# MasonFeurer/VoxelRayTracing

Hardware: AMD Instinct MI355X
Metric: Mrays/s at 1920x1080, 1 primary + 1 shadow ray (higher is better)
Workload: dtype f32

## Files before the change

bindings/rust/vrt-sys/src/lib.rs:

```rust
#![allow(non_camel_case_types)]
use std::os::raw::{c_char, c_int, c_void};

#[repr(C)]
pub struct vrt_ctx {
    _private: [u8; 0],
}

pub const VRT_OK: c_int = 0;
pub const VRT_ERR_INVALID_ARG: c_int = -1;
pub const VRT_ERR_OUT_OF_RANGE: c_int = -2;
pub const VRT_ERR_DEVICE: c_int = -3;
pub const VRT_ERR_OOM: c_int = -4;
pub const VRT_ERR_STATE: c_int = -5;

#[repr(C)]
#[derive(Clone, Copy, Default)]
pub struct vrt_material {
    pub color: [f32; 3],
    pub is_empty: u32,
    pub is_liquid: u32,
    pub scatter: f32,
    pub _padding: [u32; 2],
}

// ... 396 lines not shown
    pub fn vrt_read_tone_histogram(ctx: *mut vrt_ctx, bins: *mut u32) -> c_int;
    pub fn vrt_set_sun_light(ctx: *mut vrt_ctx, opts: *const vrt_sun_light) -> c_int;
    pub fn vrt_set_camera_sampling(ctx: *mut vrt_ctx, opts: *const vrt_camera_sampling) -> c_int;
    pub fn vrt_set_lamp_light(ctx: *mut vrt_ctx, opts: *const vrt_lamp_light) -> c_int;
    pub fn vrt_get_lamp_info(ctx: *mut vrt_ctx, out: *mut vrt_lamp_info) -> c_int;
    pub fn vrt_read_lamps(ctx: *mut vrt_ctx, out: *mut vrt_lamp, cap: u32, n: *mut u32) -> c_int;
    pub fn vrt_synchronize(ctx: *mut vrt_ctx) -> c_int;
    pub fn vrt_read_output(ctx: *mut vrt_ctx, rgb: *mut f32, ids: *mut u32, rgba8: *mut u8) -> c_int;
    pub fn vrt_present(ctx: *mut vrt_ctx, crosshair: *const vrt_crosshair, screen_w: u32, screen_h: u32, rgba8: *mut u8) -> c_int;
    pub fn vrt_selftest_exact_math(device: i32, n: u32, seed: u32, mismatches: *mut u64) -> c_int;
    pub fn vrt_selftest_math_values(device: i32, op: u32, n: u32, input: *const u32, out: *mut u32) -> c_int;
    pub fn vrt_present_device(ctx: *mut vrt_ctx, crosshair: *const vrt_crosshair, screen_w: u32, screen_h: u32, rgba8_device: *mut *mut c_void, bytes: *mut u64) -> c_int;
    pub fn vrt_set_presentation(ctx: *mut vrt_ctx, crosshair: *const vrt_crosshair, screen_w: u32, screen_h: u32, flags: u32) -> c_int;
    pub fn vrt_get_stats(ctx: *mut vrt_ctx, out: *mut vrt_stats) -> c_int;
    pub fn vrt_get_issue_profile(ctx: *mut vrt_ctx, out: *mut vrt_issue_profile) -> c_int;
    pub fn vrt_get_accel_info(ctx: *mut vrt_ctx, out: *mut vrt_accel_info) -> c_int;
    pub fn vrt_read_accel(ctx: *mut vrt_ctx, grid: *mut u32, bricks: *mut u16) -> c_int;
    pub fn vrt_read_march_cells(ctx: *mut vrt_ctx, cells: *mut u32, direct: *mut u32) -> c_int;
    pub fn vrt_read_tile_cost(ctx: *mut vrt_ctx, cost: *mut u32) -> c_int;
    pub fn vrt_read_tile_order(ctx: *mut vrt_ctx, order: *mut u32, dilated: *mut u32) -> c_int;
    pub fn vrt_selftest_tile_order(device: i32, cost: *const u32, tiles_x: u32, tiles_y: u32, radius: i32, order: *mut u32) -> c_int;
    pub fn vrt_get_sun_marks(ctx: *mut vrt_ctx, passes: *mut u32, min_leaf: *mut u32, lit_trips: *mut u32, lit: *mut u8) -> c_int;
    pub fn vrt_read_lit_voxels(ctx: *mut vrt_ctx, passes: *mut u32, layers: *mut u32, lit_trips: *mut u32, lit: *mut u8) -> c_int;
    pub fn vrt_get_dark_marks(ctx: *mut vrt_ctx, passes: *mut u32, count: *mut u32, used: *mut u32, dark: *mut u8) -> c_int;
    pub fn vrt_read_steps(ctx: *mut vrt_ctx, steps: *mut u32) -> c_int;
    pub fn vrt_set_stream(ctx: *mut vrt_ctx, hip_stream: *mut c_void) -> c_int;
    pub fn vrt_bind_output(ctx: *mut vrt_ctx, texels: *mut c_void) -> c_int;
    pub fn vrt_device_output(ctx: *mut vrt_ctx, texels: *mut *mut c_void, bytes: *mut u64) -> c_int;
    pub fn vrt_shard_info(ctx: *mut vrt_ctx, tiles_local: *mut u32, tiles_padded: *mut u32, tiles_total: *mut u32) -> c_int;
    pub fn vrt_assemble(ctx: *mut vrt_ctx, gathered: *const c_void, rank_stride_bytes: u64, dst: *mut c_void) -> c_int;
    pub fn vrt_assemble_compact(ctx: *mut vrt_ctx, gathered: *const c_void, rank_stride_bytes: u64, dst: *mut c_void) -> c_int;
    pub fn vrt_cast_rays(ctx: *mut vrt_ctx, queries: *const vrt_ray_query, n: u32, out: *mut vrt_ray_hit) -> c_int;
    pub fn vrt_cast_rays_device(ctx: *mut vrt_ctx, queries_device: *const c_void, n: u32, out_device: *mut c_void) -> c_int;
    pub fn vrt_clip_moves(ctx: *mut vrt_ctx, queries: *const vrt_box_query, n: u32, out: *mut vrt_box_move) -> c_int;
    pub fn vrt_clip_moves_device(ctx: *mut vrt_ctx, queries_device: *const c_void, n: u32, out_device: *mut c_void) -> c_int;
    pub fn vrt_get_voxels(ctx: *mut vrt_ctx, pos: *const i32, n: u32, out: *mut vrt_voxel_at) -> c_int;
    pub fn vrt_get_voxels_device(ctx: *mut vrt_ctx, pos_device: *const c_void, n: u32, out_device: *mut c_void) -> c_int;
    pub fn vrt_column_tops(ctx: *mut vrt_ctx, queries: *const vrt_column_query, n: u32, out: *mut vrt_column_top) -> c_int;
    pub fn vrt_column_tops_device(ctx: *mut vrt_ctx, queries_device: *const c_void, n: u32, out_device: *mut c_void) -> c_int;
    pub fn vrt_read_top_map(ctx: *mut vrt_ctx, flags: u32, map: *mut vrt_top_entry) -> c_int;
    pub fn vrt_top_map_device(ctx: *mut vrt_ctx, flags: u32, map_device: *mut c_void) -> c_int;
    pub fn vrt_generate_chunks(ctx: *mut vrt_ctx, seed: u32, chunk_pos: *const i32, n: u32, nodes: *mut u16, cap_nodes: u64,
                               offsets: *mut u64) -> c_int;
    pub fn vrt_build_chunks(ctx: *mut vrt_ctx, dense: *const u16, n: u32, nodes: *mut u16, cap_nodes: u64, offsets: *mut u64) -> c_int;
    pub fn vrt_edit_chunks(ctx: *mut vrt_ctx, chunk_pos: *const i32, n: u32, nodes_in: *const u16, offsets_in: *const u64,
                           shapes: *const vrt_shape, m: u32, nodes_out: *mut u16, cap_nodes: u64, offsets_out: *mut u64,
// ... 33 lines not shown
```

include/vrt.h:

```cpp
#ifndef VRT_H
#define VRT_H

#include <stdint.h>

#ifdef __cplusplus
extern "C" {
#endif

typedef struct vrt_ctx vrt_ctx;

typedef enum {
    VRT_OK = 0,
    VRT_ERR_INVALID_ARG = -1,
    VRT_ERR_OUT_OF_RANGE = -2,
    VRT_ERR_DEVICE = -3,
    VRT_ERR_OOM = -4,
    VRT_ERR_STATE = -5
} vrt_status;

typedef struct {
    float color[3];
    uint32_t is_empty;
    uint32_t is_liquid;
    float scatter;
// ... 272 lines not shown
int vrt_selftest_math_values(int32_t device, uint32_t op, uint32_t n, const uint32_t *in, uint32_t *out);

typedef struct {
    uint32_t available;
    uint32_t world_size_chunks;
    uint64_t cells;
    uint64_t bricks;
    uint64_t bytes;
    uint32_t builds;
    float last_build_ms;
    uint32_t chunk_builds;
    uint32_t ordered_frames;
} vrt_accel_info;
int vrt_get_accel_info(vrt_ctx *ctx, vrt_accel_info *out);

int vrt_read_accel(vrt_ctx *ctx, uint32_t *grid, uint16_t *bricks);

int vrt_read_march_cells(vrt_ctx *ctx, uint32_t *cells, uint32_t *direct);

int vrt_get_sun_marks(vrt_ctx *ctx, uint32_t *passes, uint32_t *min_leaf, uint32_t *lit_trips, uint8_t *lit);

int vrt_read_lit_voxels(vrt_ctx *ctx, uint32_t *passes, uint32_t *layers, uint32_t *lit_trips, uint8_t *lit);

int vrt_get_dark_marks(vrt_ctx *ctx, uint32_t *passes, uint32_t *count, uint32_t *used, uint8_t *dark);

int vrt_read_tile_cost(vrt_ctx *ctx, uint32_t *cost);

int vrt_read_tile_order(vrt_ctx *ctx, uint32_t *order, uint32_t *dilated);

int vrt_selftest_tile_order(int32_t device, const uint32_t *cost, uint32_t tiles_x, uint32_t tiles_y, int32_t radius, uint32_t *order);

int vrt_read_steps(vrt_ctx *ctx, uint32_t *steps);


typedef struct {
    float start[3];
    float max_dist;
    float dir[3];
    uint32_t _reserved;
} vrt_ray_query;

#define VRT_RAY_MISS 0u
#define VRT_RAY_HIT 1u
#define VRT_RAY_REJECTED 2u
typedef struct {
    int32_t pos[3];
// ... 116 lines not shown
```

voxelraytracing_amd/_ffi.py:

```python
from __future__ import annotations

import ctypes as C
import os

import numpy as np

_HERE = os.path.dirname(os.path.abspath(__file__))


class Material(C.Structure):
    _fields_ = [("color", C.c_float * 3), ("is_empty", C.c_uint32), ("is_liquid", C.c_uint32),
                ("scatter", C.c_float), ("_padding", C.c_uint32 * 2)]


class CamData(C.Structure):
    _fields_ = [("pos", C.c_float * 3), ("_padding0", C.c_uint32), ("inv_view_mat", C.c_float * 16),
                ("inv_proj_mat", C.c_float * 16), ("proj_size", C.c_float * 2), ("_padding1", C.c_uint32 * 2)]


class WorldData(C.Structure):
    _fields_ = [("min", C.c_int32 * 3), ("size", C.c_uint32), ("size_in_chunks", C.c_uint32),
                ("_padding", C.c_uint32 * 3)]


# ... 199 lines not shown
    "vrt_read_guide": (C.c_int, [_P, _P]),
    "vrt_set_tone_map": (C.c_int, [_P, C.POINTER(ToneMap)]),
    "vrt_get_tone_info": (C.c_int, [_P, C.POINTER(ToneInfo)]),
    "vrt_read_tone_histogram": (C.c_int, [_P, _P]),
    "vrt_set_sun_light": (C.c_int, [_P, C.POINTER(SunLight)]),
    "vrt_set_camera_sampling": (C.c_int, [_P, C.POINTER(CameraSampling)]),
    "vrt_set_lamp_light": (C.c_int, [_P, C.POINTER(LampLight)]),
    "vrt_get_lamp_info": (C.c_int, [_P, C.POINTER(LampInfo)]),
    "vrt_read_lamps": (C.c_int, [_P, _P, C.c_uint32, C.POINTER(C.c_uint32)]),
    "vrt_synchronize": (C.c_int, [_P]),
    "vrt_read_output": (C.c_int, [_P, _P, _P, _P]),
    "vrt_present": (C.c_int, [_P, C.POINTER(Crosshair), C.c_uint32, C.c_uint32, _P]),
    "vrt_selftest_exact_math": (C.c_int, [C.c_int32, C.c_uint32, C.c_uint32, C.POINTER(C.c_uint64)]),
    "vrt_selftest_math_values": (C.c_int, [C.c_int32, C.c_uint32, C.c_uint32, _P, _P]),
    "vrt_present_device": (C.c_int, [_P, C.POINTER(Crosshair), C.c_uint32, C.c_uint32, C.POINTER(_P), C.POINTER(C.c_uint64)]),
    "vrt_set_presentation": (C.c_int, [_P, C.POINTER(Crosshair), C.c_uint32, C.c_uint32, C.c_uint32]),
    "vrt_get_stats": (C.c_int, [_P, C.POINTER(Stats)]),
    "vrt_get_issue_profile": (C.c_int, [_P, C.POINTER(IssueProfile)]),
    "vrt_get_accel_info": (C.c_int, [_P, C.POINTER(AccelInfo)]),
    "vrt_read_accel": (C.c_int, [_P, _P, _P]),
    "vrt_read_march_cells": (C.c_int, [_P, _P, _P]),
    "vrt_get_sun_marks": (C.c_int, [_P, _P, _P, _P, _P]),
    "vrt_read_lit_voxels": (C.c_int, [_P, _P, _P, _P, _P]),
    "vrt_get_dark_marks": (C.c_int, [_P, _P, _P, _P, _P]),
    "vrt_read_tile_cost": (C.c_int, [_P, _P]),
    "vrt_read_tile_order": (C.c_int, [_P, _P, C.POINTER(C.c_uint32)]),
    "vrt_selftest_tile_order": (C.c_int, [C.c_int32, _P, C.c_uint32, C.c_uint32, C.c_int32, _P]),
    "vrt_read_steps": (C.c_int, [_P, _P]),
    "vrt_set_stream": (C.c_int, [_P, _P]),
    "vrt_bind_output": (C.c_int, [_P, _P]),
    "vrt_device_output": (C.c_int, [_P, C.POINTER(_P), C.POINTER(C.c_uint64)]),
    "vrt_shard_info": (C.c_int, [_P, C.POINTER(C.c_uint32), C.POINTER(C.c_uint32), C.POINTER(C.c_uint32)]),
    "vrt_assemble": (C.c_int, [_P, _P, C.c_uint64, _P]),
    "vrt_assemble_compact": (C.c_int, [_P, _P, C.c_uint64, _P]),
    "vrt_cast_rays": (C.c_int, [_P, _P, C.c_uint32, _P]),
    "vrt_cast_rays_device": (C.c_int, [_P, _P, C.c_uint32, _P]),
    "vrt_clip_moves": (C.c_int, [_P, _P, C.c_uint32, _P]),
    "vrt_clip_moves_device": (C.c_int, [_P, _P, C.c_uint32, _P]),
    "vrt_get_voxels": (C.c_int, [_P, _P, C.c_uint32, _P]),
    "vrt_get_voxels_device": (C.c_int, [_P, _P, C.c_uint32, _P]),
    "vrt_column_tops": (C.c_int, [_P, _P, C.c_uint32, _P]),
    "vrt_column_tops_device": (C.c_int, [_P, _P, C.c_uint32, _P]),
    "vrt_read_top_map": (C.c_int, [_P, C.c_uint32, _P]),
    "vrt_top_map_device": (C.c_int, [_P, C.c_uint32, _P]),
    "vrt_generate_chunks": (C.c_int, [_P, C.c_uint32, _P, C.c_uint32, _P, C.c_uint64, _P]),
    "vrt_build_chunks": (C.c_int, [_P, _P, C.c_uint32, _P, C.c_uint64, _P]),
# ... 200 lines not shown
```

voxelraytracing_amd/csrc/vrt_ctx.h:

```cpp
#pragma once
#include <hip/hip_runtime.h>

#include <algorithm>
#include <array>
#include <atomic>
#include <condition_variable>
#include <functional>
#include <memory>
#include <mutex>
#include <thread>
#include <cmath>
#include <cstdarg>
#include <cstdio>
#include <cstdlib>
#include <cstring>
#include <new>
#include <string>
#include <vector>

#include "vrt_devbuf.h"
#include "vrt_frame_plan.h"
#include "vrt_handle.h"
#include "vrt_device.h"

// ... 194 lines not shown
        uint64_t gen = 0;
        struct SunMarks {
            struct Key {
                uint64_t gen = 0;
                float sun[3] = {0.f, 0.f, 0.f};
                uint32_t min_lo = 0;
                uint32_t liquid[8] = {0, 0, 0, 0, 0, 0, 0, 0};
                bool same(const Key &o) const {
                    return gen == o.gen && memcmp(sun, o.sun, sizeof sun) == 0 && min_lo == o.min_lo && memcmp(liquid, o.liquid, sizeof liquid) == 0;
                }
            } made, want;
            uint32_t want_frames = 0;
            bool valid = false;
            Buf<uint16_t> d_pool;
            Buf<uint32_t> d_clash;
            bool voxels_valid = false;
            uint64_t pool_gen = ~0ull;
            Pinned h_clash;
            bool clash_pending = false;
            uint64_t clash_gen = ~0ull;
            uint32_t voxel_layers = 0;
            Buf<uint8_t> d_floors;
            bool dark_valid = false;
            Event ev;
            bool pending = false;
            hipStream_t stream = nullptr;
            Event ev_guard;
            bool holds(uint64_t gen) const { return valid && made.gen == gen; }
            bool pool_fits(size_t entries) const { return d_pool && d_pool.cap() == entries; }
            bool pool_is_of(uint64_t gen, size_t entries) const { return pool_gen == gen && holds(gen) && pool_fits(entries); }
            void take_from(const SunMarks &A, uint64_t a_gen, uint64_t gen) {
                valid = A.holds(a_gen);
                made = A.made; made.gen = gen;
                pending = voxels_valid = false;
                dark_valid = valid && A.dark_valid;
            }
        } lit;
        Event ev_updated;
        bool update_pending = false;
    };
    Tables tabs[kMaxInFlight];
    uint64_t tables_gen = 0;
    bool tables_split = false;
    uint32_t quiet_frames = 0;
    bool shared_readers_in_flight = false;
    Buf<uint32_t> d_brick_total;
// ... 3 lines not shown
    uint32_t n_bricks = 0;
    uint32_t accel_S = 0;
    bool accel_dirty = true;
    bool accel_ok = false;
    uint32_t accel_max_s = 0;
    uint32_t timing_every = 8, frame_no = 0;
    bool path_pool = true;
    bool path_cells = true;
    uint32_t path_samples = 8;
    uint32_t path_pool_batches = 0;
    uint32_t path_refill = 0;
    uint32_t accel_builds = 0;
    bool sun_marks = true;
    uint32_t lit_slab = 0;
    uint32_t lit_passes = 0;
    bool lit_voxels = true;
    int lit_voxel_layers = -1;
    uint32_t lit_voxel_passes = 0;
    uint32_t lit_last_voxel_layers = 0, lit_last_voxel_trips = 0;
    uint32_t lit_last_min_leaf = 0, lit_last_trips = 0;
    bool dark_marks = true;
    int dark_depth = -1;
    uint32_t dark_passes = 0;
    bool dark_last_used = false;
    bool tile_lpt = true;
    uint32_t view_gen = 0;
    uint32_t frame_view_gen = ~0u;
    uint32_t order_view_gen = ~0u;
    uint32_t tile_lpt_moving = 1;
    uint32_t order_uses = 0;
    uint32_t mov_backoff = 0, mov_skip = 0;
    bool mov_any_size = false;
    uint32_t mov_radius = 5;
    uint32_t one_w = 0, one_h = 0;
    bool one_to_one = false;
    bool pres_on = false;
    vrt_crosshair pres_ch{};
    uint32_t pres_w = 0, pres_h = 0, pres_flags = 0;
    uint32_t pres_for_w = 0, pres_for_h = 0, pres_box[4] = {0, 0, 0, 0};
    bool pres_fusable = false;
    uint32_t ordered_frames = 0;
    bool order_dilated = false;
    uint32_t cam_gen = 0, order_cam_gen = 0;
    vrt_cam_data order_cam{};
    bool tile_order_stale = false;
    uint32_t frame_mode = ~0u;
// ... 290 lines not shown
```

voxelraytracing_amd/csrc/vrt_device.h:

```cpp
#pragma once

#include <hip/hip_runtime.h>
#include <stddef.h>
#include <stdint.h>

#include "../../include/vrt.h"

namespace vrt {

constexpr float kShadowBias = 0.002f;
constexpr float kShadowFactor = 0.35f;
constexpr uint32_t kMaxSteps = 500u;
constexpr uint32_t kIdNormYNeg = 1u << 23;

constexpr uint32_t kCamNotFinite = 1u, kCamOnPlane = 2u, kCamOutside = 4u;

constexpr uint32_t kAirLeaf = 0xFF800000u;
__host__ __device__ inline bool is_split_entry(uint32_t e) { return (int32_t)e < 0 && e < kAirLeaf; }
constexpr uint32_t kAirUnlit = 1u << 22;
constexpr uint32_t kLitBelow = kAirLeaf | kAirUnlit;
constexpr uint32_t kAirDark = 1u << 21;
constexpr uint32_t kLitVoxel = 0x7FFFu;
__host__ __device__ inline uint32_t grid_entry(uint32_t x) { return x - 1u < 31u ? (kAirLeaf | kAirUnlit | x) : x; }

using Texel = uint4;

constexpr uint32_t kMaterials = 256u;
__host__ __device__ inline const float *emission_table(const vrt_material *mats) { return reinterpret_cast<const float *>(mats + kMaterials); }
__host__ __device__ inline const vrt_polish *polish_table(const vrt_material *mats) {
    return reinterpret_cast<const vrt_polish *>(emission_table(mats) + kMaterials);
}
static_assert(sizeof(vrt_polish) == 32 && (kMaterials * (sizeof(vrt_material) + sizeof(float))) % 16 == 0, "the polish table's entries are 16-byte aligned");
__host__ __device__ inline const vrt_translucency *translucency_table(const vrt_material *mats) {
    return reinterpret_cast<const vrt_translucency *>(polish_table(mats) + kMaterials);
}
__host__ __device__ inline const uint32_t *coat_word(const vrt_material *mats) {
    return reinterpret_cast<const uint32_t *>(translucency_table(mats) + kMaterials);
}
static_assert(sizeof(vrt_translucency) == 16, "a translucency entry is one 16-byte load");

struct FrameParams {
    const uint16_t *nodes;
    const uint32_t *roots;
    const vrt_material *mats;
    const uint32_t *grid;
// ... 174 lines not shown
```

voxelraytracing_amd/csrc/vrt_frames.hip:

```cpp
#include "vrt_ctx.h"

thread_local std::string g_create_err;

int fail(vrt_ctx *ctx, int code, const char *fmt, ...) {
    char buf[512];
    va_list ap;
    va_start(ap, fmt);
    vsnprintf(buf, sizeof buf, fmt, ap);
    va_end(ap);
    if (ctx) ctx->err = buf;
    else g_create_err = buf;
    return code;
}

vrt_host_prof g_host_prof;

int quiesce(vrt_ctx *c) {
    if (c->alt_pending) {
        for (hipStream_t st : c->extra_stream)
            if (st) HIP_TRY(c, hipStreamSynchronize(st));
        c->alt_pending = false;
    }
    if (c->own_pending) {
        HIP_TRY(c, hipStreamSynchronize(c->own_stream));
// ... 438 lines not shown
    c->shard_rank = cfg->shard_rank;
    c->shard_count = sc;
    c->shard_w0 = cfg->shard_root_weight ? cfg->shard_root_weight : 1u;
    c->tile_major = (sc > 1u && !(cfg->flags & VRT_FLAG_ROW_MAJOR)) || (cfg->flags & VRT_FLAG_TILE_MAJOR);
    c->compact = (cfg->flags & VRT_FLAG_COMPACT) != 0;
    c->width = cfg->width;
    c->height = cfg->height;
    c->max_nodes = cfg->max_nodes & ~1u;
    c->accel_max_s = kAccelMaxS;
    if (const char *e = getenv("VRT_ACCEL_MAX_S")) {
        const long v = strtol(e, nullptr, 10);
        if (v >= 0 && v < (long)kAccelMaxS) c->accel_max_s = (uint32_t)v;
    }
    c->march_direct_max_s = kMarchDirectMaxS;
    if (const char *e = getenv("VRT_MARCH_DIRECT_MAX_S")) {
        const long v = strtol(e, nullptr, 10);
        if (v >= 0 && v <= (long)kMarchDirectMaxS) c->march_direct_max_s = (uint32_t)v;
    }
    if (const char *e = getenv("VRT_TILE_ORDER")) c->tile_lpt = e[0] != '0';
    if (const char *e = getenv("VRT_SUN_MARKS")) c->sun_marks = e[0] != '0';
    if (const char *e = getenv("VRT_LIT_VOXELS")) c->lit_voxels = e[0] != '0';
    if (const char *e = getenv("VRT_LIT_VOXEL_LAYERS")) { const long v = atol(e); if (v >= 0 && v <= 4096) c->lit_voxel_layers = (int)v; }
    if (const char *e = getenv("VRT_DARK_MARKS")) c->dark_marks = e[0] != '0';
    if (const char *e = getenv("VRT_DARK_DEPTH")) { const long v = atol(e); if (v >= 0 && v <= 4096) c->dark_depth = (int)v; }
    if (const char *e = getenv("VRT_LIT_SLAB")) { const long v = atol(e); if (v >= 1 && v <= 4096) c->lit_slab = (uint32_t)v; }
    if (const char *e = getenv("VRT_TILE_ORDER_MOVING")) c->tile_lpt_moving = e[0] != '0' ? 1u : 0u;
    c->mov_any_size = getenv("VRT_TILE_ORDER_MOVING") != nullptr;
    if (const char *e = getenv("VRT_TILE_ORDER_RADIUS")) { const int v = atoi(e); if (v >= 1 && v <= 6) c->mov_radius = (uint32_t)v; }
    if (const char *e = getenv("VRT_PATH_POOL")) c->path_pool = e[0] != '0';
    if (const char *e = getenv("VRT_LAMP_CAP")) { const long v = atol(e); if (v >= 1 && v <= (1l << 24)) c->lamp_cap = (uint32_t)v; }
    if (const char *e = getenv("VRT_TONE_BLOCKS")) { const long v = atol(e); if (v >= 1 && v <= 65536) c->tone_blocks = (uint32_t)v; }
    if (const char *e = getenv("VRT_PATH_CELLS")) c->path_cells = e[0] != '0';
    if (const char *e = getenv("VRT_PATH_POOL_REFILL")) c->path_refill = (uint32_t)atoi(e);
    if (const char *e = getenv("VRT_PATH_POOL_K")) { const int v = atoi(e); if (v == 4 || v == 5) c->path_pool_batches = (uint32_t)v; }
    if (const char *e = getenv("VRT_PATH_SAMPLES_PER_CHAIN")) { const int v = atoi(e); if (v >= 1 && v <= 16) c->path_samples = (uint32_t)v; }
    if (const char *e = getenv("VRT_TIMING_EVERY")) { const long v = strtol(e, nullptr, 10); if (v >= 1 && v <= 1000000) c->timing_every = (uint32_t)v; }
    memset(c->h_mats, 0, sizeof c->h_mats);
    memset(c->h_emission, 0, sizeof c->h_emission);
    memset(c->h_polish, 0, sizeof c->h_polish);
    memset(c->h_translucency, 0, sizeof c->h_translucency);
    memset(&c->cam, 0, sizeof c->cam);
    memset(&c->settings, 0, sizeof c->settings);
    memset(&c->world, 0, sizeof c->world);
    memset(&c->stats, 0, sizeof c->stats);

    auto body = [&]() -> int {
// ... 507 lines not shown
```

voxelraytracing_amd/csrc/vrt_lit.hip:

```cpp
#include "vrt_ctx.h"

namespace vrt {

namespace {

struct LitPass {
    uint32_t G;
    uint32_t axis;
    uint32_t up;
    uint32_t min_lo;
    float sun[3];
};

__device__ inline bool lit_reach(float c4, float s_min, float s_max, float r_lo, float r_hi, float allow, uint32_t G, uint32_t *lo, uint32_t *hi) {
    const float b_lo = c4 + (s_min < 0.0f ? r_hi : r_lo) * s_min - allow;
    const float b_hi = c4 + 4.0f + (s_max > 0.0f ? r_hi : r_lo) * s_max + allow;
    int l = (int)floorf(b_lo * 0.25f), h = (int)floorf(b_hi * 0.25f);
    const int own = (int)(c4 * 0.25f);
    if (!(s_min < 0.0f)) l = max(l, own);
    if (!(s_max > 0.0f)) h = min(h, own);
    if (h < 0 || l >= (int)G) return false;
    *lo = (uint32_t)max(l, 0);
    *hi = (uint32_t)min(h, (int)G - 1);
    return true;
// ... 243 lines not shown
        const double r_lo = k >= 2u ? 4.0 * (double)k - 5.0 : 0.0, r_hi = 4.0 * (double)k + 5.0;
        const double allow = fmin(0.015 * (double)(k + 1u), 1.0) + 0.01;
        int ul, uh, vl, vh;
        if (!dark_reach(u4, us_min, us_max, r_lo, r_hi, allow, (int)G, &ul, &uh) || !dark_reach(v4, vs_min, vs_max, r_lo, r_hi, allow, (int)G, &vl, &vh))
            break;
        if (k == 0u) continue;
        uint32_t m = 15u;
        for (int nv = vl; nv <= vh; nv++)
            for (int nu = ul; nu <= uh; nu++) m &= floors[layer + (size_t)nu * su + (size_t)nv * sv];
        if (m) { dark = true; break; }
    }
    grid[at] = dark ? ((e & ~kAirUnlit) | kAirDark) : ((e & ~kAirDark) | kAirUnlit);
}

void launch_accel_dark(uint32_t *grid, const uint16_t *bricks, uint32_t entries, uint8_t *floors, uint32_t G, uint32_t axis, bool up, const float sun[3],
                       uint32_t depth, const uint32_t liquid[8], hipStream_t st) {
    DarkPass dp{G, axis, up ? 1u : 0u, depth, {sun[0], sun[1], sun[2]}, {}};
    for (int i = 0; i < 8; i++) dp.liquid[i] = liquid[i];
    const uint32_t blocks = (G * G * G + 255u) / 256u;
    hipLaunchKernelGGL(accel_floor_masks_kernel, dim3(blocks), dim3(256), 0, st, grid, bricks, entries, floors, dp);
    hipLaunchKernelGGL(accel_dark_kernel, dim3(blocks), dim3(256), 0, st, grid, floors, dp);
}

}

}

namespace {

using Tables = vrt_ctx::Tables;
using SunMarks = Tables::SunMarks;

struct LitPlan { uint32_t axis; bool up; uint32_t min_lo, trips; };
constexpr uint32_t kLitSettleFrames = 4;
bool lit_plan(uint32_t world_size, const float sun[3], LitPlan *lp) {
    for (int k = 0; k < 3; k++)
        if (!std::isfinite(sun[k])) return false;
    const float lo = -1.0f, hi = (float)world_size + 1.0f;
    float best = 0.0f;
    for (uint32_t a = 0; a < 3; a++)
        for (int up = 0; up < 2; up++) {
            const float clear = up ? sun[a] - hi : lo - sun[a];
            if (clear > best) { best = clear; lp->axis = a; lp->up = up != 0; }
        }
    if (!(best > 0.0f)) return false;
    for (uint32_t b = 0; b < 3; b++) {
// ... 4 lines not shown
    for (uint32_t L = 4u; L <= 32u; L *= 2u) {
        const uint32_t B = 6u * (world_size / L + 1u) + 2u;
        if (B + 2u <= vrt::kMaxSteps) { lp->min_lo = L - 1u; lp->trips = vrt::kMaxSteps - B - 1u; return true; }
    }
    return false;
}

uint32_t lit_slab_depth(const vrt_ctx *c, uint32_t G) {
    const uint32_t depth = c->lit_slab ? c->lit_slab : G <= 64u ? G : G <= 128u ? 32u : 8u;
    return depth < G ? depth : G;
}

uint32_t lit_voxel_layers(const vrt_ctx *c, uint32_t G) {
    if (!c->lit_voxels) return 0u;
    if (c->lit_voxel_layers >= 0) return (uint32_t)c->lit_voxel_layers;
    return G <= 64u ? 8u : 0u;
}
uint32_t lit_voxel_budget(uint32_t layers) { return 2u * (3u * layers + 6u); }

uint32_t dark_depth(const vrt_ctx *c, uint32_t G) {
    if (!c->dark_marks) return 0u;
    const uint32_t depth = c->dark_depth >= 0 ? (uint32_t)c->dark_depth : G <= 64u ? 32u : 0u;
    return depth < G ? depth : G;
}

bool settled(SunMarks &L, const SunMarks::Key &now) {
    if (!(L.want_frames && L.want.same(now))) { L.want = now; L.want_frames = 0u; }
    if (++L.want_frames < kLitSettleFrames) return false;
    L.want_frames = 0u;
    return true;
}

int order_pass(vrt_ctx *c, SunMarks &L, uint32_t k, hipStream_t st, bool shares) {
    if (k == 0u && (shares || c->shared_readers_in_flight)) {
        VRT_TRY(quiesce_before_frame(c));
        if (st != c->stream) {
            HIP_TRY(c, L.ev_guard.ensure());
            HIP_TRY(c, hipEventRecord(L.ev_guard, c->stream));
            HIP_TRY(c, hipStreamWaitEvent(st, L.ev_guard, 0));
        }
    }
    if (L.pending && L.stream != st) HIP_TRY(c, hipStreamWaitEvent(st, L.ev, 0));
    return VRT_OK;
}

int launch_passes(vrt_ctx *c, Tables &T, const LitPlan &lp, const SunMarks::Key &now, hipStream_t st) {
    SunMarks &L = T.lit;
    const uint32_t G = c->accel_S * 8u;
    L.valid = L.voxels_valid = false;
    vrt::launch_accel_lit(T.d_grid, G, lp.axis, lp.up, lp.min_lo, now.sun, lit_slab_depth(c, G), st);
    HIP_TRY(c, hipGetLastError());
    const uint32_t layers = lit_voxel_layers(c, G);
    L.clash_pending = false;
    if (layers && c->liquid_is_range && lit_voxel_budget(layers) < lp.trips && T.d_bricks.cap() >= 64u && L.clash_gen != T.gen) {
        HIP_TRY(c, L.d_pool.exactly(T.d_bricks.cap()));
        HIP_TRY(c, L.d_clash.once(1));
        HIP_TRY(c, L.h_clash.ensure((size_t)64));
        vrt::launch_accel_lit_voxels(T.d_grid, T.d_bricks, L.d_pool, (uint32_t)T.d_bricks.cap(), G, lp.axis, lp.up, now.sun, layers, L.d_clash, st);
        HIP_TRY(c, hipGetLastError());
        HIP_TRY(c, hipMemcpyAsync(L.h_clash, L.d_clash, sizeof(uint32_t), hipMemcpyDeviceToHost, st));
        L.clash_pending = true;
        L.pool_gen = T.gen;
        L.voxels_valid = true;
        L.voxel_layers = layers;
        c->lit_voxel_passes += 1u;
    }
    L.dark_valid = false;
    if (const uint32_t depth = dark_depth(c, G)) {
        HIP_TRY(c, L.d_floors.exactly(T.d_grid.cap()));
        vrt::launch_accel_dark(T.d_grid, T.d_bricks, (uint32_t)T.d_bricks.cap(), L.d_floors, G, lp.axis, lp.up, now.sun, depth, now.liquid, st);
        HIP_TRY(c, hipGetLastError());
        L.dark_valid = true;
        c->dark_passes += 1u;
    }
    HIP_TRY(c, L.ev.ensure());
    HIP_TRY(c, hipEventRecord(L.ev, st));
    L.pending = true;
    L.stream = st;
    L.valid = true;
    L.made = now;
    c->lit_passes += 1u;
    return VRT_OK;
}

int hand_out(vrt_ctx *c, Tables &T, const LitPlan &lp, hipStream_t st, vrt::FrameParams &P) {
    SunMarks &L = T.lit;
    if (L.pending && L.stream != st) {
        if (hipEventQuery(L.ev) == hipSuccess) L.pending = false;
        else HIP_TRY(c, hipStreamWaitEvent(st, L.ev, 0));
    }
    P.shadow_below = vrt::kLitBelow;
    P.lit_trips = lp.trips;
    c->lit_last_min_leaf = lp.min_lo + 1u;
    c->lit_last_trips = lp.trips;
    c->dark_last_used = L.dark_valid;
    if (L.clash_pending && hipEventQuery(L.ev) == hipSuccess) {
        L.clash_pending = false;
        if (*reinterpret_cast<volatile uint32_t *>(L.h_clash.get())) { L.voxels_valid = false; L.clash_gen = T.gen; }
    }
    if (L.voxels_valid && L.pool_fits(T.d_bricks.cap()) && lit_voxel_budget(L.voxel_layers) < lp.trips) {
        P.shadow_bricks = L.d_pool;
        P.lit_voxel_trips = lp.trips - lit_voxel_budget(L.voxel_layers);
        c->lit_last_voxel_layers = L.voxel_layers;
        c->lit_last_voxel_trips = P.lit_voxel_trips;
    }
    return VRT_OK;
}

int ensure_sun_marks(vrt_ctx *c, uint32_t k, hipStream_t st, bool shares, vrt::FrameParams &P) {
    Tables &T = c->tabs[k];
    LitPlan lp{};
    if (!c->accel_ok || !T.live || !T.d_grid || !lit_plan(c->world.size, P.sun_local, &lp)) return VRT_OK;
    SunMarks::Key now{T.gen, {P.sun_local[0], P.sun_local[1], P.sun_local[2]}, lp.min_lo, {}};
    if (dark_depth(c, c->accel_S * 8u)) memcpy(now.liquid, c->liquid_mask, sizeof now.liquid);
    if (T.lit.valid && T.lit.made.same(now)) {
        T.lit.want_frames = 0u;
    } else {
        if (!settled(T.lit, now)) return VRT_OK;
        VRT_TRY(order_pass(c, T.lit, k, st, shares));
        VRT_TRY(launch_passes(c, T, lp, now, st));
    }
    return hand_out(c, T, lp, st, P);
}

int marks_of_last_frame(vrt_ctx *c, const char *who, std::vector<uint32_t> &cells) {
    if (!c->accel_ok || c->accel_dirty || !c->tabs[c->last.tab].live)
        return fail(c, VRT_ERR_STATE, "%s: the tables are not up to date (render a frame first)", who);
    HIP_TRY(c, hipSetDevice(c->device));
    QUIESCE(c);
    HIP_TRY(c, hipStreamSynchronize(c->stream));
    Tables &T = c->tabs[c->last.tab];
    if (T.lit.pending) { HIP_TRY(c, hipEventSynchronize(T.lit.ev)); T.lit.pending = false; }
    cells.resize((size_t)c->accel_S * c->accel_S * c->accel_S * 512u);
    return read_grid_cells(c, T.d_grid, cells.data());
}

}

int sun_marks_for_frame(vrt_ctx *c, uint32_t tab, hipStream_t st, bool shares, vrt::FrameParams &P) {
    c->lit_last_min_leaf = c->lit_last_trips = c->lit_last_voxel_layers = c->lit_last_voxel_trips = 0u;
    c->dark_last_used = false;
    return c->sun_marks ? ensure_sun_marks(c, tab, st, shares, P) : VRT_OK;
}

extern "C" {

int vrt_get_sun_marks(vrt_ctx *c, uint32_t *passes, uint32_t *min_leaf, uint32_t *lit_trips, uint8_t *lit) {
    GRP_ROOT(c, vrt_get_sun_marks(d, passes, min_leaf, lit_trips, lit));
    if (!c) return VRT_ERR_INVALID_ARG;
    if (passes) *passes = c->lit_passes;
    if (min_leaf) *min_leaf = c->lit_last_min_leaf;
    if (lit_trips) *lit_trips = c->lit_last_trips;
    if (!lit) return VRT_OK;
    std::vector<uint32_t> cells;
    VRT_TRY(marks_of_last_frame(c, "vrt_get_sun_marks", cells));
    const bool held = c->tabs[c->last.tab].lit.holds(c->tabs[c->last.tab].gen);
    for (size_t i = 0; i < cells.size(); i++) lit[i] = (held && cells[i] >= vrt::kAirLeaf && !(cells[i] & (vrt::kAirUnlit | vrt::kAirDark))) ? 1u : 0u;
    return VRT_OK;
}

int vrt_get_dark_marks(vrt_ctx *c, uint32_t *passes, uint32_t *count, uint32_t *used, uint8_t *dark) {
    GRP_ROOT(c, vrt_get_dark_marks(d, passes, count, used, dark));
    if (!c) return VRT_ERR_INVALID_ARG;
    if (passes) *passes = c->dark_passes;
// ... 21 lines not shown
    if (lit_trips) *lit_trips = c->lit_last_voxel_trips;
    if (!lit) return VRT_OK;
    std::vector<uint32_t> cells;
    VRT_TRY(marks_of_last_frame(c, "vrt_read_lit_voxels", cells));
    const Tables &T = c->tabs[c->last.tab];
    const size_t G = (size_t)c->accel_S * 8u, W = G * 4u;
    memset(lit, 0, W * W * W);
    if (!T.lit.pool_is_of(T.gen, T.d_bricks.cap())) return VRT_OK;
    std::vector<uint16_t> pool(T.lit.d_pool.cap());
    HIP_TRY(c, hipMemcpy(pool.data(), T.lit.d_pool, pool.size() * sizeof(uint16_t), hipMemcpyDeviceToHost));
    for (size_t z = 0; z < G; z++)
        for (size_t y = 0; y < G; y++)
            for (size_t x = 0; x < G; x++) {
                const uint32_t e = cells[(z * G + y) * G + x];
                const size_t at = e & 0x7FFFFFC0u;
                if (!vrt::is_split_entry(e) || at + 64u > pool.size()) continue;
                for (size_t u = 0; u < 64u; u++)
                    if ((uint32_t)(pool[at + u] >> 1) == vrt::kLitVoxel)
                        lit[((z * 4u + (u >> 4)) * W + (y * 4u + ((u >> 2) & 3u))) * W + (x * 4u + (u & 3u))] = 1u;
            }
    return VRT_OK;
}

}
```

voxelraytracing_amd/csrc/vrt_march.h:

```cpp
#pragma once

#include "vrt_device.h"


namespace vrt {

__device__ __forceinline__ int trunc2i(float x) {
    int r;
    asm("v_cvt_i32_f32 %0, %1" : "=v"(r) : "v"(x));
    return r;
}

constexpr uint32_t kBandLo = 0x30800000u;
constexpr uint32_t kBandSpan = 0x4E800000u - kBandLo;
__device__ __forceinline__ bool in_band(float x) { return (__float_as_uint(x) & 0x7FFFFFFFu) - kBandLo <= kBandSpan; }
__device__ __forceinline__ bool in_band3(V3 v) {
    const uint32_t a = (__float_as_uint(v.x) & 0x7FFFFFFFu) - kBandLo, b = (__float_as_uint(v.y) & 0x7FFFFFFFu) - kBandLo,
                   c = (__float_as_uint(v.z) & 0x7FFFFFFFu) - kBandLo;
    return max(max(a, b), c) <= kBandSpan;
}
__device__ __forceinline__ float rcp_refined(float d) {
    const float r = __builtin_amdgcn_rcpf(d);
    const float e = __builtin_fmaf(-d, r, 1.0f);
    return __builtin_fmaf(e, r, r);
// ... 566 lines not shown
    constexpr uint32_t kTwo23 = 0x4B000000u;
    uint32_t mxm = kTwo23 | (mx ? 0x001FFFFFu : 0u), mym = kTwo23 | (my ? 0x001FFFFFu : 0u), mzm = kTwo23 | (mz ? 0x001FFFFFu : 0u);
    float cx = mx ? -8388607.0f : -8388608.0f, cy = my ? -8388607.0f : -8388608.0f, cz = mz ? -8388607.0f : -8388608.0f;
    asm("" : "+v"(mxm), "+v"(mym), "+v"(mzm));

    const uint32_t wsize = P.world.size;
    constexpr bool kLitStops = SHADOW && !STATS;
    const TableBuf gb = table_buffer(P.grid, P.grid_bytes), bb_plain = table_buffer(P.bricks, P.brick_bytes);
    const TableBuf bb16_plain = __builtin_amdgcn_make_buffer_rsrc(const_cast<uint16_t *>(P.bricks), 2, P.brick_bytes / 2u, 0x00020000);
    const TableBuf bb_lit = table_buffer(P.shadow_bricks, P.brick_bytes);
    const TableBuf bb16_lit = __builtin_amdgcn_make_buffer_rsrc(const_cast<uint16_t *>(P.shadow_bricks), 2, P.brick_bytes / 2u, 0x00020000);
    uint32_t liq_lo = P.liquid_lo, liq_span = P.liquid_span;
    if (!P.liquid_is_range) { liq_lo = 1u; liq_span = 0xFFFFFFFEu; }
    else if (liq_lo == 0u) { if (liq_span) { liq_lo = 1u; liq_span -= 1u; } else liq_lo = 0x80000000u; }
    const uint32_t row_bytes = (P.grid_dim + 1u) * 4u, slab_bytes = (P.grid_dim + 1u) * row_bytes;

    int vx = trunc2i(pos.x), vy = trunc2i(pos.y), vz = trunc2i(pos.z);
    uint32_t voxel = 0u;
    float step = -1.0f, adx = 0.0f, ady = 0.0f, adz = 0.0f;
    float dew = -1.0f;
    constexpr uint32_t kSlow = 0xFFFFFFFFu;
    uint32_t plain_below = kLitStops ? P.shadow_below : kAirLeaf;
    const uint32_t cells_limit = (kLitStops && plain_below != kAirLeaf) ? P.lit_trips : kMaxSteps;
    bool lit_voxels = kLitStops && LITVOX && P.shadow_bricks != nullptr && P.lit_voxel_trips < cells_limit;
    uint32_t limit = lit_voxels ? P.lit_voxel_trips : cells_limit;
    bool lit_stop = false, dark_stop = false;
    uint32_t slow_below = careful ? kSlow : plain_below;
    float total_len = 0.0f;
    uint32_t iter = 0u;
    uint32_t looked_up = 0u;

    auto take_step = [&](uint32_t sel) __attribute__((always_inline)) {
        const float tx = (__uint_as_float(bfi(sel, mxm, (uint32_t)vx)) + cx) - pos.x;
        const float ty = (__uint_as_float(bfi(sel, mym, (uint32_t)vy)) + cy) - pos.y;
        const float tz = (__uint_as_float(bfi(sel, mzm, (uint32_t)vz)) + cz) - pos.z;
        adx = abs_mul(tx, ux);
        ady = abs_mul(ty, uy);
        adz = abs_mul(tz, uz);
        step = min3_f32(adx, ady, adz);
        if (__ballot(!(step > 0.0f)) != 0ull)
            step = __uint_as_float(min3_u32(__float_as_uint(adx) - 1u, __float_as_uint(ady) - 1u, __float_as_uint(adz) - 1u) + 1u);
        total_len += step;
        const float sp = step + 0.001f;
        pos.x += dir.x * (step == adx ? sp : step);
        pos.y += dir.y * (step == ady ? sp : step);
        pos.z += dir.z * (step == adz ? sp : step);
        vx = flr2i(pos.x);
// ... 220 lines not shown
```

voxelraytracing_amd/graphics.py:

```python
from __future__ import annotations

import ctypes as C
from typing import Optional

import numpy as np

from . import _ffi
from ._ffi import (CamData, Material, Settings, WorldData, Stats, RenderOpts,
                   MODE_PRIMARY, MODE_PRIMARY_SHADOW, MODE_PATH, RENDER_OWN_STREAMS, RENDER_TIMED, RENDER_ACCUMULATE)


class VrtError(RuntimeError):
    def __init__(self, code: int, msg: str):
        super().__init__(f"vrt error {code}: {msg}")
        self.code = code


def _f(vals, n):
    return (C.c_float * n)(*[float(v) for v in vals])


_scratch3a, _scratch3b, _scratch2 = (C.c_float * 3)(), (C.c_float * 3)(), (C.c_float * 2)()


# ... 283 lines not shown
    def read_tile_cost(self, tiles: int) -> np.ndarray:
        cost = np.empty(tiles, dtype=np.uint32)
        self._ck(self._lib.vrt_read_tile_cost(self._h, cost.ctypes.data_as(C.c_void_p)))
        return cost

    def read_tile_order(self, tiles: int):
        order = np.empty(tiles, dtype=np.uint32)
        dilated = C.c_uint32()
        self._ck(self._lib.vrt_read_tile_order(self._h, order.ctypes.data_as(C.c_void_p), C.byref(dilated)))
        return order, bool(dilated.value)

    def lit_voxels(self, voxels: bool = False):
        p, k, t = C.c_uint32(), C.c_uint32(), C.c_uint32()
        lit = None
        if voxels:
            n = self.accel_info().world_size_chunks * 32
            lit = np.empty((n, n, n), dtype=np.uint8)
        self._ck(self._lib.vrt_read_lit_voxels(self._h, C.byref(p), C.byref(k), C.byref(t), lit.ctypes.data_as(C.c_void_p) if voxels else None))
        out = dict(passes=p.value, layers=k.value, lit_trips=t.value)
        if voxels:
            out["lit"] = lit
        return out

    def dark_marks(self, cells: bool = False):
        p, n, u = C.c_uint32(), C.c_uint32(), C.c_uint32()
        dark = None
        if cells:
            g = self.accel_info().world_size_chunks * 8
            dark = np.empty((g, g, g), dtype=np.uint8)
        self._ck(self._lib.vrt_get_dark_marks(self._h, C.byref(p), C.byref(n), C.byref(u), dark.ctypes.data_as(C.c_void_p) if cells else None))
        out = dict(passes=p.value, count=n.value, used=bool(u.value))
        if cells:
            out["dark"] = dark
        return out

    def sun_marks(self, cells: bool = False):
        p, m, t = C.c_uint32(), C.c_uint32(), C.c_uint32()
        lit = None
        if cells:
            g = self.accel_info().world_size_chunks * 8
            lit = np.empty((g, g, g), dtype=np.uint8)
        self._ck(self._lib.vrt_get_sun_marks(self._h, C.byref(p), C.byref(m), C.byref(t), lit.ctypes.data_as(C.c_void_p) if cells else None))
        out = dict(passes=p.value, min_leaf=m.value, lit_trips=t.value)
        if cells:
            out["lit"] = lit
        return out
# ... 110 lines not shown
```

Before: 69990.

## Precompute per-voxel sun-occlusion marks so shadow rays stop early in dark air

Adds a precompute kernel that walks each empty sub-voxel in split bricks toward the sun over several layers and, where every covering voxel is blocked, marks it as a dark voxel in the lit-brick pool. Shadow rays that hit such a mark can end at once instead of marching to the sky. The pass runs by default on small worlds (16 layers when G<=64) and is redone whenever the sun marks are rebuilt. It also turns off lit-voxel stops on the careful march path. It adds precompute cost, a debug readback API and bindings, and risks wrong shadows if the conservative cone bounds are too loose.

Measured after the change: 71750 (median of 6 runs). +2.5%, better.

```diff
diff --git a/bindings/rust/vrt-sys/src/lib.rs b/bindings/rust/vrt-sys/src/lib.rs
--- a/bindings/rust/vrt-sys/src/lib.rs
+++ b/bindings/rust/vrt-sys/src/lib.rs
@@ -442,6 +442,7 @@
     pub fn vrt_selftest_tile_order(device: i32, cost: *const u32, tiles_x: u32, tiles_y: u32, radius: i32, order: *mut u32) -> c_int;
     pub fn vrt_get_sun_marks(ctx: *mut vrt_ctx, passes: *mut u32, min_leaf: *mut u32, lit_trips: *mut u32, lit: *mut u8) -> c_int;
     pub fn vrt_read_lit_voxels(ctx: *mut vrt_ctx, passes: *mut u32, layers: *mut u32, lit_trips: *mut u32, lit: *mut u8) -> c_int;
+    pub fn vrt_read_dark_voxels(ctx: *mut vrt_ctx, passes: *mut u32, layers: *mut u32, dark: *mut u8) -> c_int;
     pub fn vrt_get_dark_marks(ctx: *mut vrt_ctx, passes: *mut u32, count: *mut u32, used: *mut u32, dark: *mut u8) -> c_int;
     pub fn vrt_read_steps(ctx: *mut vrt_ctx, steps: *mut u32) -> c_int;
     pub fn vrt_set_stream(ctx: *mut vrt_ctx, hip_stream: *mut c_void) -> c_int;
diff --git a/include/vrt.h b/include/vrt.h
--- a/include/vrt.h
+++ b/include/vrt.h
@@ -318,6 +318,8 @@
 
 int vrt_read_lit_voxels(vrt_ctx *ctx, uint32_t *passes, uint32_t *layers, uint32_t *lit_trips, uint8_t *lit);
 
+int vrt_read_dark_voxels(vrt_ctx *ctx, uint32_t *passes, uint32_t *layers, uint8_t *dark);
+
 int vrt_get_dark_marks(vrt_ctx *ctx, uint32_t *passes, uint32_t *count, uint32_t *used, uint8_t *dark);
 
 int vrt_read_tile_cost(vrt_ctx *ctx, uint32_t *cost);
diff --git a/voxelraytracing_amd/_ffi.py b/voxelraytracing_amd/_ffi.py
--- a/voxelraytracing_amd/_ffi.py
+++ b/voxelraytracing_amd/_ffi.py
@@ -245,6 +245,7 @@
     "vrt_read_march_cells": (C.c_int, [_P, _P, _P]),
     "vrt_get_sun_marks": (C.c_int, [_P, _P, _P, _P, _P]),
     "vrt_read_lit_voxels": (C.c_int, [_P, _P, _P, _P, _P]),
+    "vrt_read_dark_voxels": (C.c_int, [_P, _P, _P, _P]),
     "vrt_get_dark_marks": (C.c_int, [_P, _P, _P, _P, _P]),
     "vrt_read_tile_cost": (C.c_int, [_P, _P]),
     "vrt_read_tile_order": (C.c_int, [_P, _P, C.POINTER(C.c_uint32)]),
diff --git a/voxelraytracing_amd/csrc/vrt_ctx.h b/voxelraytracing_amd/csrc/vrt_ctx.h
--- a/voxelraytracing_amd/csrc/vrt_ctx.h
+++ b/voxelraytracing_amd/csrc/vrt_ctx.h
@@ -240,6 +240,7 @@
             uint32_t voxel_layers = 0;
             Buf<uint8_t> d_floors;
             bool dark_valid = false;
+            uint32_t dark_voxel_layers = 0;
             Event ev;
             bool pending = false;
             hipStream_t stream = nullptr;
@@ -289,6 +290,9 @@
     bool dark_marks = true;
     int dark_depth = -1;
     uint32_t dark_passes = 0;
+    int dark_voxel_layers = -1;
+    uint32_t dark_voxel_passes = 0;
+    uint32_t dark_last_voxel_layers = 0;
     bool dark_last_used = false;
     bool tile_lpt = true;
     uint32_t view_gen = 0;
diff --git a/voxelraytracing_amd/csrc/vrt_device.h b/voxelraytracing_amd/csrc/vrt_device.h
--- a/voxelraytracing_amd/csrc/vrt_device.h
+++ b/voxelraytracing_amd/csrc/vrt_device.h
@@ -21,6 +21,7 @@
 constexpr uint32_t kLitBelow = kAirLeaf | kAirUnlit;
 constexpr uint32_t kAirDark = 1u << 21;
 constexpr uint32_t kLitVoxel = 0x7FFFu;
+constexpr uint32_t kDarkVoxel = 0x7FFEu;
 __host__ __device__ inline uint32_t grid_entry(uint32_t x) { return x - 1u < 31u ? (kAirLeaf | kAirUnlit | x) : x; }
 
 using Texel = uint4;
diff --git a/voxelraytracing_amd/csrc/vrt_frames.hip b/voxelraytracing_amd/csrc/vrt_frames.hip
--- a/voxelraytracing_amd/csrc/vrt_frames.hip
+++ b/voxelraytracing_amd/csrc/vrt_frames.hip
@@ -484,6 +484,7 @@
     if (const char *e = getenv("VRT_LIT_VOXELS")) c->lit_voxels = e[0] != '0';
     if (const char *e = getenv("VRT_LIT_VOXEL_LAYERS")) { const long v = atol(e); if (v >= 0 && v <= 4096) c->lit_voxel_layers = (int)v; }
     if (const char *e = getenv("VRT_DARK_MARKS")) c->dark_marks = e[0] != '0';
+    if (const char *e = getenv("VRT_DARK_VOXEL_LAYERS")) { const long v = atol(e); if (v >= 0 && v <= 4096) c->dark_voxel_layers = (int)v; }
     if (const char *e = getenv("VRT_DARK_DEPTH")) { const long v = atol(e); if (v >= 0 && v <= 4096) c->dark_depth = (int)v; }
     if (const char *e = getenv("VRT_LIT_SLAB")) { const long v = atol(e); if (v >= 1 && v <= 4096) c->lit_slab = (uint32_t)v; }
     if (const char *e = getenv("VRT_TILE_ORDER_MOVING")) c->tile_lpt_moving = e[0] != '0' ? 1u : 0u;
diff --git a/voxelraytracing_amd/csrc/vrt_lit.hip b/voxelraytracing_amd/csrc/vrt_lit.hip
--- a/voxelraytracing_amd/csrc/vrt_lit.hip
+++ b/voxelraytracing_amd/csrc/vrt_lit.hip
@@ -289,6 +289,108 @@
     hipLaunchKernelGGL(accel_dark_kernel, dim3(blocks), dim3(256), 0, st, grid, floors, dp);
 }
 
+struct DarkVoxelPass {
+    uint32_t G, axis, up;
+    uint32_t layers;
+    uint32_t entries;
+    float sun[3];
+    uint32_t liquid[8];
+};
+
+__device__ inline bool dark_voxel_reach(double i, double s_min, double s_max, double r_lo, double r_hi, double allow, int W, int *lo, int *hi) {
+    const double b_lo = i + (s_min < 0.0 ? r_hi : r_lo) * s_min - allow;
+    const double b_hi = i + 1.0 + (s_max > 0.0 ? r_hi : r_lo) * s_max + allow;
+    int l = (int)floor(b_lo), h = (int)floor(b_hi);
+    const int own = (int)i;
+    if (!(s_min < 0.0)) l = max(l, own);
+    if (!(s_max > 0.0)) h = min(h, own);
+    *lo = l;
+    *hi = h;
+    return l >= 0 && h < W;
+}
+
+__device__ inline bool dark_voxel_walk(const uint32_t *grid, const uint16_t *bricks, const DarkVoxelPass &dp, int ia, int iu, int iv, uint32_t ca,
+                                       uint32_t cu, uint32_t cv, uint32_t ha, uint32_t hu, uint32_t hv) {
+    const int W = (int)(dp.G * 4u);
+    const uint32_t a = dp.axis, u = a == 0u ? 1u : 0u, v = a == 2u ? 1u : 2u;
+    const double fa = (double)ia, fu = (double)iu, fv = (double)iv;
+    const double sun_a = dp.up ? (double)dp.sun[a] : (double)W - (double)dp.sun[a], sun_u = (double)dp.sun[u], sun_v = (double)dp.sun[v];
+    const double d_lo = sun_a - (fa + 2.0), d_hi = sun_a - (fa - 1.0);
+    double us_min, us_max, vs_min, vs_max;
+    dark_slopes(sun_u - (fu + 2.0), sun_u - (fu - 1.0), d_lo, d_hi, &us_min, &us_max);
+    dark_slopes(sun_v - (fv + 2.0), sun_v - (fv - 1.0), d_lo, d_hi, &vs_min, &vs_max);
+    auto blocks = [&](uint32_t voxel) {
+        const uint32_t id = voxel < 255u ? voxel : 255u;
+        return voxel != 0u && !((dp.liquid[id >> 5] >> (id & 31u)) & 1u);
+    };
+    bool inside = true, dark = false;
+    for (uint32_t k = 0; k <= dp.layers && inside && !dark; k++) {
+        const int la = ia + (int)k;
+        const double r_lo = k >= 2u ? (double)k - 2.0 : 0.0, r_hi = (double)k + 2.0;
+        const double allow = fmin(0.015 * (double)(k + 1u), 1.0) + 0.01;
+        int ul, uh, vl, vh;
+        const bool in_u = dark_voxel_reach(fu, us_min, us_max, r_lo, r_hi, allow, W, &ul, &uh);
+        const bool in_v = dark_voxel_reach(fv, vs_min, vs_max, r_lo, r_hi, allow, W, &vl, &vh);
+        inside = in_u && in_v && la < W;
+        if (!inside || k == 0u) continue;
+        const uint32_t qa = (uint32_t)(dp.up ? la : W - 1 - la);
+        const uint32_t cell_a = (qa >> 2) * ca, bit_a = (qa & 3u) << ha;
+        bool shut = true;
+        for (int nv = vl; nv <= vh && shut; nv++)
+            for (int nu = ul; nu <= uh && shut; nu++) {
+                const uint32_t e = grid[cell_a + ((uint32_t)nu >> 2) * cu + ((uint32_t)nv >> 2) * cv];
+                if (e >= kAirLeaf) {
+                    shut = (e & kAirDark) != 0u;
+                } else if (is_split_entry(e)) {
+                    const uint32_t at = (e & 0x7FFFFFC0u) + (bit_a | (((uint32_t)nu & 3u) << hu) | (((uint32_t)nv & 3u) << hv));
+                    shut = at < dp.entries && blocks((uint32_t)bricks[at] >> 1);
+                } else {
+                    shut = e != 0u && blocks(e >> 16);
+                }
+            }
+        dark = shut;
+    }
+    return dark;
+}
+
+__global__ void __launch_bounds__(256) accel_dark_voxels_kernel(const uint32_t *grid, const uint16_t *bricks, uint16_t *lit_bricks, DarkVoxelPass dp,
+                                                                const uint32_t *clash) {
+    if (*clash != 0u) return;
+    const uint32_t G = dp.G, G1 = G + 1u, lane = threadIdx.x & 63u;
+    const uint32_t cells = G * G * G, waves = (cells + kLitVoxelCellsPerWave - 1u) / kLitVoxelCellsPerWave;
+    const uint32_t wave = (blockIdx.x * blockDim.x + threadIdx.x) >> 6;
+    if (wave >= waves) return;
+    const uint32_t mine = wave + lane * waves;
+    uint32_t e_mine = 0u;
+    if (lane < kLitVoxelCellsPerWave && mine < cells) e_mine = grid[(((mine / G) % G) * G1 + mine / (G * G)) * G1 + mine % G];
+    const uint32_t a = dp.axis, u = a == 0u ? 1u : 0u, v = a == 2u ? 1u : 2u;
+    const uint32_t cs[3] = {1u, G1, G1 * G1};
+    const uint32_t ca = cs[a], cu = cs[u], cv = cs[v], ha = 2u * a, hu = 2u * u, hv = 2u * v;
+    const int W = (int)(G * 4u);
+    unsigned long long todo = __ballot(is_split_entry(e_mine));
+    while (todo) {
+        const uint32_t i = (uint32_t)__ffsll((long long)todo) - 1u;
+        todo &= todo - 1ull;
+        const uint32_t e = (uint32_t)__shfl((int)e_mine, (int)i, 64), cell = wave + i * waves;
+        if ((e & 0x7FFFFFC0u) + 64u > dp.entries) continue;
+        const uint32_t at = (e & 0x7FFFFFC0u) + lane;
+        const int px = (int)((cell % G) * 4u + (lane & 3u)), py = (int)((cell / (G * G)) * 4u + ((lane >> 2) & 3u)), pz = (int)(((cell / G) % G) * 4u + (lane >> 4));
+        const int pa = a == 0u ? px : a == 1u ? py : pz, pu = u == 0u ? px : py, pv = v == 1u ? py : pz;
+        const uint32_t b = bricks[at];
+        if ((b >> 1) == 0u && ((uint32_t)lit_bricks[at] >> 1) != kLitVoxel &&
+            dark_voxel_walk(grid, bricks, dp, dp.up ? pa : W - 1 - pa, pu, pv, ca, cu, cv, ha, hu, hv))
+            lit_bricks[at] = (uint16_t)((kDarkVoxel << 1) | (b & 1u));
+    }
+}
+
+void launch_accel_dark_voxels(const uint32_t *grid, const uint16_t *bricks, uint16_t *lit_bricks, uint32_t entries, uint32_t G, uint32_t axis, bool up,
+                              const float sun[3], uint32_t layers, const uint32_t liquid[8], const uint32_t *clash, hipStream_t st) {
+    DarkVoxelPass dp{G, axis, up ? 1u : 0u, layers, entries, {sun[0], sun[1], sun[2]}, {}};
+    for (int i = 0; i < 8; i++) dp.liquid[i] = liquid[i];
+    const uint32_t waves = (G * G * G + kLitVoxelCellsPerWave - 1u) / kLitVoxelCellsPerWave;
+    hipLaunchKernelGGL(accel_dark_voxels_kernel, dim3((waves + 3u) / 4u), dim3(256), 0, st, grid, bricks, lit_bricks, dp, clash);
+}
+
 }
 
 }
@@ -339,6 +441,11 @@
     if (!c->dark_marks) return 0u;
     const uint32_t depth = c->dark_depth >= 0 ? (uint32_t)c->dark_depth : G <= 64u ? 32u : 0u;
     return depth < G ? depth : G;
+}
+
+uint32_t dark_voxel_layers(const vrt_ctx *c, uint32_t G) {
+    if (c->dark_voxel_layers >= 0) return (uint32_t)c->dark_voxel_layers;
+    return G <= 64u ? 16u : 0u;
 }
 
 bool settled(SunMarks &L, const SunMarks::Key &now) {
@@ -382,6 +489,7 @@
         L.voxel_layers = layers;
         c->lit_voxel_passes += 1u;
     }
+    const bool pool_made = L.voxels_valid;
     L.dark_valid = false;
     if (const uint32_t depth = dark_depth(c, G)) {
         HIP_TRY(c, L.d_floors.exactly(T.d_grid.cap()));
@@ -389,6 +497,13 @@
         HIP_TRY(c, hipGetLastError());
         L.dark_valid = true;
         c->dark_passes += 1u;
+    }
+    L.dark_voxel_layers = 0u;
+    if (const uint32_t layers = pool_made ? dark_voxel_layers(c, G) : 0u) {
+        vrt::launch_accel_dark_voxels(T.d_grid, T.d_bricks, L.d_pool, (uint32_t)T.d_bricks.cap(), G, lp.axis, lp.up, now.sun, layers, c->liquid_mask, L.d_clash, st);
+        HIP_TRY(c, hipGetLastError());
+        L.dark_voxel_layers = layers;
+        c->dark_voxel_passes += 1u;
     }
     HIP_TRY(c, L.ev.ensure());
     HIP_TRY(c, hipEventRecord(L.ev, st));
@@ -420,6 +535,7 @@
         P.lit_voxel_trips = lp.trips - lit_voxel_budget(L.voxel_layers);
         c->lit_last_voxel_layers = L.voxel_layers;
         c->lit_last_voxel_trips = P.lit_voxel_trips;
+        c->dark_last_voxel_layers = L.dark_voxel_layers;
     }
     return VRT_OK;
 }
@@ -429,7 +545,8 @@
     LitPlan lp{};
     if (!c->accel_ok || !T.live || !T.d_grid || !lit_plan(c->world.size, P.sun_local, &lp)) return VRT_OK;
     SunMarks::Key now{T.gen, {P.sun_local[0], P.sun_local[1], P.sun_local[2]}, lp.min_lo, {}};
-    if (dark_depth(c, c->accel_S * 8u)) memcpy(now.liquid, c->liquid_mask, sizeof now.liquid);
+    if (dark_depth(c, c->accel_S * 8u) || (lit_voxel_layers(c, c->accel_S * 8u) && dark_voxel_layers(c, c->accel_S * 8u)))
+        memcpy(now.liquid, c->liquid_mask, sizeof now.liquid);
     if (T.lit.valid && T.lit.made.same(now)) {
         T.lit.want_frames = 0u;
     } else {
@@ -457,6 +574,7 @@
 int sun_marks_for_frame(vrt_ctx *c, uint32_t tab, hipStream_t st, bool shares, vrt::FrameParams &P) {
     c->lit_last_min_leaf = c->lit_last_trips = c->lit_last_voxel_layers = c->lit_last_voxel_trips = 0u;
     c->dark_last_used = false;
+    c->dark_last_voxel_layers = 0u;
     return c->sun_marks ? ensure_sun_marks(c, tab, st, shares, P) : VRT_OK;
 }
 
@@ -524,4 +642,32 @@
     return VRT_OK;
 }
 
-}
+int vrt_read_dark_voxels(vrt_ctx *c, uint32_t *passes, uint32_t *layers, uint8_t *dark) {
+    GRP_ROOT(c, vrt_read_dark_voxels(d, passes, layers, dark));
+    if (!c) return VRT_ERR_INVALID_ARG;
+    if (passes) *passes = c->dark_voxel_passes;
+    if (layers) *layers = c->dark_last_voxel_layers;
+    if (!dark) return VRT_OK;
+    std::vector<uint32_t> cells;
+    VRT_TRY(marks_of_last_frame(c, "vrt_read_dark_voxels", cells));
+    const Tables &T = c->tabs[c->last.tab];
+    const size_t G = (size_t)c->accel_S * 8u, W = G * 4u;
+    memset(dark, 0, W * W * W);
+    if (!T.lit.pool_is_of(T.gen, T.d_bricks.cap())) return VRT_OK;
+    std::vector<uint16_t> pool(T.lit.d_pool.cap()), plain(T.d_bricks.cap());
+    HIP_TRY(c, hipMemcpy(pool.data(), T.lit.d_pool, pool.size() * sizeof(uint16_t), hipMemcpyDeviceToHost));
+    HIP_TRY(c, hipMemcpy(plain.data(), T.d_bricks, plain.size() * sizeof(uint16_t), hipMemcpyDeviceToHost));
+    for (size_t z = 0; z < G; z++)
+        for (size_t y = 0; y < G; y++)
+            for (size_t x = 0; x < G; x++) {
+                const uint32_t e = cells[(z * G + y) * G + x];
+                const size_t at = e & 0x7FFFFFC0u;
+                if (!vrt::is_split_entry(e) || at + 64u > pool.size()) continue;
+                for (size_t u = 0; u < 64u; u++)
+                    if ((uint32_t)(pool[at + u] >> 1) == vrt::kDarkVoxel && (plain[at + u] >> 1) == 0u)
+                        dark[((z * 4u + (u >> 4)) * W + (y * 4u + ((u >> 2) & 3u))) * W + (x * 4u + (u & 3u))] = 1u;
+            }
+    return VRT_OK;
+}
+
+}
diff --git a/voxelraytracing_amd/csrc/vrt_march.h b/voxelraytracing_amd/csrc/vrt_march.h
--- a/voxelraytracing_amd/csrc/vrt_march.h
+++ b/voxelraytracing_amd/csrc/vrt_march.h
@@ -612,7 +612,7 @@
     constexpr uint32_t kSlow = 0xFFFFFFFFu;
     uint32_t plain_below = kLitStops ? P.shadow_below : kAirLeaf;
     const uint32_t cells_limit = (kLitStops && plain_below != kAirLeaf) ? P.lit_trips : kMaxSteps;
-    bool lit_voxels = kLitStops && LITVOX && P.shadow_bricks != nullptr && P.lit_voxel_trips < cells_limit;
+    bool lit_voxels = kLitStops && LITVOX && !careful && P.shadow_bricks != nullptr && P.lit_voxel_trips < cells_limit;
     uint32_t limit = lit_voxels ? P.lit_voxel_trips : cells_limit;
     bool lit_stop = false, dark_stop = false;
     uint32_t slow_below = careful ? kSlow : plain_below;
diff --git a/voxelraytracing_amd/graphics.py b/voxelraytracing_amd/graphics.py
--- a/voxelraytracing_amd/graphics.py
+++ b/voxelraytracing_amd/graphics.py
@@ -329,6 +329,18 @@
             out["lit"] = lit
         return out
 
+    def dark_voxels(self, voxels: bool = False):
+        p, k = C.c_uint32(), C.c_uint32()
+        dark = None
+        if voxels:
+            n = self.accel_info().world_size_chunks * 32
+            dark = np.empty((n, n, n), dtype=np.uint8)
+        self._ck(self._lib.vrt_read_dark_voxels(self._h, C.byref(p), C.byref(k), dark.ctypes.data_as(C.c_void_p) if voxels else None))
+        out = dict(passes=p.value, layers=k.value)
+        if voxels:
+            out["dark"] = dark
+        return out
+
     def dark_marks(self, cells: bool = False):
         p, n, u = C.c_uint32(), C.c_uint32(), C.c_uint32()
         dark = None
```
